# PhucNguyenAH/tacotron2_subword

Measured on AMD Instinct MI355X. Metric: mel_frames_per_sec_train, higher is better.
Workload: dtype bf16; 1 GPU; BERT_Tacotron2 default hparams (SMA), full training iteration fwd+loss+bwd+clip+Adam, B=64/GPU, 100 phones, 60 sub-word tokens, 400 frames, 80-mel; global_batch=64, frames_per_item=400, parallelism=dp1, torch_ops=loss reductions, cat/transpose copies, persistent_chains=True, recurrent_steps_bf16=True

## Files before the change

### include/t2amd.h

```cpp
#ifndef T2AMD_H
#define T2AMD_H
#include <stddef.h>
#include <stdint.h>

#ifdef __cplusplus
extern "C" {
#endif

#define T2_ATTN_SMA 0
#define T2_ATTN_LSA 1
#define T2_ATTN_DCA 4
#define T2_ATTN_GMM 3
#define T2_ATTN_FWD2 2

enum {
    T2_SITE_PRENET1 = 1, T2_SITE_PRENET2 = 2, T2_SITE_PRENET1_SUB = 3, T2_SITE_PRENET2_SUB = 4,
    T2_SITE_ATT_H = 5, T2_SITE_ATT_C = 6, T2_SITE_ATT_H_SUB = 7, T2_SITE_ATT_C_SUB = 8,
    T2_SITE_DEC_H = 9, T2_SITE_DEC_C = 10, T2_SITE_NOISE = 11, T2_SITE_NOISE_SUB = 12,
    T2_SITE_ENC0 = 16,
    T2_SITE_ENCSUB0 = 20,
    T2_SITE_POSTNET0 = 24
};

const char* t2_last_error(void);
#define T2_ABI_VERSION 4
int t2_version(void);
int t2_chain_status(uint32_t* out_host );
int t2_chain_status_clear(void);
int t2_debug_report_abort(uint32_t code, void* stream);
int t2_debug_occupy(int workgroups, int milliseconds, void* stream);
int t2_chain_claimed(void);
int t2_set_precision(int mode);
int t2_get_precision(void);
int t2_gemm_counts(uint64_t* out_host , int reset);
int t2_set_gemm_split_min_mflop(int mflop);
int t2_set_split_steps(int on);
int t2_get_split_steps(void);
int t2_step_counts(uint64_t* out_host , int reset);
int t2_set_overlap(int on);
int t2_set_chain(int on);
int t2_get_chain(void);
int t2_set_chain_bwd(int on);
int t2_set_gemm_staging(int on);
int t2_set_gemm_fold(int on);
int t2_set_bn_fuse(int on);
int t2_get_bn_fuse(void);
int t2_bn_fuse_counts(uint64_t* out_host , int reset);
int t2_side_join(void* stream);
int t2_defer_counts(uint64_t* out_host , int reset);

typedef struct t2_dims {
    int n_mel;
    int prenet_dim;
    int enc_dim;
    int att_rnn_dim;
    int dec_rnn_dim;
    int att_dim;
    int loc_filters;
    int loc_kernel;
    int attention_kind;
    float p_att_dropout, p_dec_dropout, p_prenet_dropout;
    int n_streams;
    float score_mask_value, score_mask_value_sub;
    int score_mask_given;
} t2_dims;

typedef struct t2_attention_weights {
    const float* wq;
    const float* wm;
    const float* v;
    const float* loc_conv;
    const float* loc_dense;
    const float* mlp_b1;
    const float* mlp_w2;
    const float* mlp_b2;
    const float* dca_T;
    const float* dca_bT;
    const float* dca_P;
} t2_attention_weights;
typedef struct t2_lstm_weights { const float *w_ih, *w_hh, *b_ih, *b_hh; } t2_lstm_weights;
typedef struct t2_decoder_weights {
    const float *prenet_w1, *prenet_w2;
    const float *prenet_sub_w1, *prenet_sub_w2;
    t2_lstm_weights att, att_sub;
    t2_attention_weights attn, attn_sub;
    t2_lstm_weights dec;
    const float *proj_w, *proj_b;
    const float *gate_w, *gate_b;
} t2_decoder_weights;

typedef struct t2_decoder_layout {
    size_t total_floats;
    size_t x, p1, p2, p1s, p2s;
    size_t pm, pms;
    size_t prea, preas;
    size_t ga, gas;
    size_t cna, cnas, ca, cas;
// ... 622 lines not shown
```

### tacotron2_subword_amd/_lib.py

```python
from __future__ import annotations

import ctypes as C
import os

import torch

_HERE = os.path.dirname(os.path.abspath(__file__))
LIB_PATH = os.environ.get("T2AMD_LIB") or os.path.join(_HERE, "libt2amd.so")

ATTN_SMA, ATTN_LSA, ATTN_FWD2, ATTN_GMM, ATTN_DCA = 0, 1, 2, 3, 4

SITE = dict(PRENET1=1, PRENET2=2, PRENET1_SUB=3, PRENET2_SUB=4, ATT_H=5, ATT_C=6, ATT_H_SUB=7, ATT_C_SUB=8,
            DEC_H=9, DEC_C=10, NOISE=11, NOISE_SUB=12, ENC0=16, ENCSUB0=20, POSTNET0=24)

_fp = C.POINTER(C.c_float)
_ip = C.POINTER(C.c_int32)


class Dims(C.Structure):
    _fields_ = [("n_mel", C.c_int), ("prenet_dim", C.c_int), ("enc_dim", C.c_int), ("att_rnn_dim", C.c_int),
                ("dec_rnn_dim", C.c_int), ("att_dim", C.c_int), ("loc_filters", C.c_int), ("loc_kernel", C.c_int),
                ("attention_kind", C.c_int), ("p_att_dropout", C.c_float), ("p_dec_dropout", C.c_float),
                ("p_prenet_dropout", C.c_float), ("n_streams", C.c_int),
                ("score_mask_value", C.c_float), ("score_mask_value_sub", C.c_float), ("score_mask_given", C.c_int)]
# ... 361 lines not shown
class WaveglowBackwardArgs(C.Structure):
    _fields_ = [("B", C.c_int), ("T", C.c_int), ("n_mel", C.c_int), ("n_samples", C.c_long), ("packed", C.c_void_p), ("packed_bwd", C.c_void_p),
                ("saved", C.c_void_p), ("mel", C.c_void_p), ("audio", C.c_void_p), ("dz", C.c_void_p), ("dlog_s_host", C.POINTER(C.c_void_p)),
                ("workspace", C.c_void_p), ("grad", C.c_void_p), ("kernel_ms_host", C.POINTER(C.c_double))]


class WaveglowWeightGradArgs(C.Structure):
    _fields_ = [("B", C.c_int), ("M", C.c_int), ("nc", C.c_int), ("n_cond", C.c_int), ("L", C.c_int), ("taps", C.c_int), ("d", C.c_int),
                ("a_rows", C.c_int), ("x_rows", C.c_int),
                ("a", C.c_void_p), ("x", C.c_void_p), ("spect", C.c_void_p), ("dw_x", C.c_void_p), ("dw_spect", C.c_void_p), ("db", C.c_void_p),
                ("workspace", C.c_void_p), ("db2", C.c_void_p)]


class WaveglowStartBackwardArgs(C.Structure):
    _fields_ = [("B", C.c_int), ("nc", C.c_int), ("c", C.c_int), ("n_half", C.c_int), ("L", C.c_int), ("dx", C.c_void_p), ("w_start", C.c_void_p),
                ("audio_in", C.c_void_p), ("d_in", C.c_void_p), ("dw_start", C.c_void_p), ("db_start", C.c_void_p), ("workspace", C.c_void_p)]


class WaveglowHeadBackwardArgs(C.Structure):
    _fields_ = [("B", C.c_int), ("n_group", C.c_int), ("n_samples", C.c_long), ("d_in", C.c_void_p), ("audio", C.c_void_p), ("part", C.c_void_p),
                ("dw", C.c_void_p)]


class WaveglowGateBackwardArgs(C.Structure):
    _fields_ = [("B", C.c_int), ("nc", C.c_int), ("L", C.c_int), ("last", C.c_int), ("dx", C.c_void_p), ("d_out", C.c_void_p), ("w_rs", C.c_void_p),
                ("t", C.c_void_p), ("g", C.c_void_p), ("packed_ws", C.c_void_p), ("du", C.c_void_p), ("acts", C.c_void_p)]


class WaveglowConvBackwardArgs(C.Structure):
    _fields_ = [("B", C.c_int), ("nc", C.c_int), ("n_cond", C.c_int), ("L", C.c_int), ("d", C.c_int), ("first_dx", C.c_int), ("first_spect", C.c_int),
                ("du", C.c_void_p), ("w_in", C.c_void_p), ("w_cond", C.c_void_p), ("packed_ws", C.c_void_p), ("dx", C.c_void_p), ("d_spect", C.c_void_p)]


class WaveglowTailBackwardArgs(C.Structure):
    _fields_ = [("B", C.c_int), ("nc", C.c_int), ("n_half", C.c_int), ("L", C.c_int), ("n_peel", C.c_int), ("n_group", C.c_int), ("z_offset", C.c_int),
                ("out", C.c_void_p), ("w_end", C.c_void_p), ("b_end", C.c_void_p), ("audio_in", C.c_void_p), ("w_next", C.c_void_p), ("d_next", C.c_void_p),
                ("dz", C.c_void_p), ("dlog_s", C.c_void_p), ("d_out", C.c_void_p), ("d_in", C.c_void_p), ("part", C.c_void_p), ("dw_end", C.c_void_p),
                ("db_end", C.c_void_p), ("dw_next", C.c_void_p)]


class WaveglowUpsampleBackwardArgs(C.Structure):
    _fields_ = [("B", C.c_int), ("n_mel", C.c_int), ("T", C.c_int), ("n_group", C.c_int), ("n_samples", C.c_long),
                ("mel", C.c_void_p), ("d_spect", C.c_void_p), ("dw", C.c_void_p), ("db", C.c_void_p)]


WAVEGLOW_KERNELS = ("upsample", "start", "gated_conv", "res_skip", "couple")
WAVEGLOW_FORWARD_KERNELS = ("upsample", "start", "gated_conv", "res_skip", "head", "tail", "sums")
WAVEGLOW_BACKWARD_KERNELS = ("tail_backward", "gate_backward", "conv_backward", "cond_backward", "weight_grad", "weight_grad_reduce", "start_backward",
                             "upsample_backward")
WAVEGLOW_GATED, WAVEGLOW_RES_SKIP, WAVEGLOW_UPSAMPLE = 0, 1, 2

ABI_VERSION = 4

EXPORTS = ["t2_last_error", "t2_version", "t2_chain_status", "t2_chain_status_clear", "t2_debug_report_abort", "t2_debug_occupy", "t2_chain_claimed", "t2_set_precision", "t2_get_precision", "t2_gemm_counts", "t2_set_gemm_split_min_mflop", "t2_set_split_steps", "t2_get_split_steps", "t2_step_counts", "t2_set_overlap", "t2_set_chain", "t2_get_chain", "t2_set_chain_bwd", "t2_set_gemm_staging", "t2_set_gemm_fold", "t2_set_bn_fuse", "t2_get_bn_fuse", "t2_bn_fuse_counts", "t2_side_join", "t2_defer_counts", "t2_decoder_layout_query", "t2_decoder_forward", "t2_decoder_infer",
           "t2_decoder_bwd_layout_query", "t2_decoder_backward", "t2_decoder_pass_plan", "t2_prof_enable", "t2_prof_collect", "t2_adam_chunks", "t2_adam_step", "t2_adam_norm",
           "t2_conv_bn_forward", "t2_conv_bn_backward", "t2_embedding_forward", "t2_embedding_backward",
           "t2_lstm_seq_forward", "t2_lstm_seq_backward", "t2_lstm_seq_chain_ws_floats", "t2_gemm_ex", "t2_prof_gemm", "t2_gemm_plan", "t2_chain_plan", "t2_conv_handoff_plan", "t2_colsum", "t2_mask_btc",
           "t2_finalize_bct", "t2_mask_bt", "t2_gemm", "t2_rng_keep_mask", "t2_rng_normal",
           "t2_softdtw_plan", "t2_softdtw_dist", "t2_softdtw_forward", "t2_softdtw_backward", "t2_softdtw_dist_backward",
           "t2_ssim_plan", "t2_ssim_forward", "t2_ssim_backward",
           "t2_hifigan_plan", "t2_hifigan_pack", "t2_hifigan_forward", "t2_vocoder_packed_floats", "t2_vocoder_conv1d", "t2_vocoder_conv_transpose1d",
           "t2_stft_plan", "t2_stft_pack", "t2_stft_analysis", "t2_stft_synthesis", "t2_melspec_plan", "t2_melspec_pack", "t2_melspec",
           "t2_waveglow_plan", "t2_waveglow_pack", "t2_waveglow_infer", "t2_waveglow_packed_floats", "t2_waveglow_gated_conv", "t2_waveglow_res_skip",
           "t2_waveglow_upsample", "t2_waveglow_couple", "t2_waveglow_forward_plan", "t2_waveglow_forward", "t2_waveglow_logdet",
           "t2_waveglow_logdet_matrices", "t2_waveglow_head", "t2_waveglow_tail",
           "t2_waveglow_backward_plan", "t2_waveglow_grad_offsets", "t2_waveglow_pack_backward", "t2_waveglow_train_forward", "t2_waveglow_backward",
           "t2_waveglow_weight_grad_ws_floats", "t2_waveglow_weight_grad", "t2_waveglow_gate_backward", "t2_waveglow_conv_backward_packed_floats",
           "t2_waveglow_conv_backward", "t2_waveglow_tail_backward", "t2_waveglow_upsample_backward", "t2_waveglow_start_backward", "t2_waveglow_head_backward"]

_lib = None


def lib() -> C.CDLL:
    global _lib
    if _lib is None:
        if not os.path.exists(LIB_PATH):
            raise RuntimeError(f"{LIB_PATH} is missing: the HIP extension must be built (see __graft_entry__.build); "
                               "there is no CPU fallback for the product path")
        L = C.CDLL(LIB_PATH)
        L.t2_last_error.restype = C.c_char_p
        if L.t2_version() != ABI_VERSION:
            raise RuntimeError(f"{LIB_PATH} speaks ABI version {L.t2_version()}, this binding {ABI_VERSION}: rebuild the library "
                               "(the argument structs differ in size between versions)")
        L.t2_chain_status.argtypes = [C.POINTER(C.c_uint32)]
        L.t2_debug_report_abort.argtypes = [C.c_uint32, C.c_void_p]
        L.t2_debug_occupy.argtypes = [C.c_int, C.c_int, C.c_void_p]
        L.t2_gemm.argtypes = [C.c_void_p, C.c_void_p, C.c_void_p, C.c_int, C.c_int, C.c_int, C.c_long, C.c_long, C.c_long,
                              C.c_long, C.c_long, C.c_void_p, C.c_int, C.c_float, C.c_float, C.c_void_p, C.c_size_t,
                              C.c_int, C.c_void_p]
        L.t2_rng_keep_mask.argtypes = [C.c_uint64, C.c_uint32, C.c_uint32, C.c_float, C.c_void_p, C.c_void_p]
        L.t2_rng_normal.argtypes = [C.c_uint64, C.c_uint32, C.c_uint32, C.c_void_p, C.c_void_p]
        L.t2_decoder_layout_query.argtypes = [C.POINTER(Dims), C.c_int, C.c_int, C.c_int, C.c_int, C.POINTER(DecoderLayout)]
        L.t2_decoder_forward.argtypes = [C.POINTER(Dims), C.POINTER(DecoderWeights), C.POINTER(DecoderFwdArgs), C.c_void_p]
        L.t2_decoder_infer.argtypes = [C.POINTER(Dims), C.POINTER(DecoderWeights), C.POINTER(DecoderInferArgs), C.c_void_p]
        L.t2_decoder_bwd_layout_query.argtypes = [C.POINTER(Dims), C.c_int, C.c_int, C.c_int, C.c_int, C.POINTER(DecoderBwdLayout)]
        L.t2_decoder_backward.argtypes = [C.POINTER(Dims), C.POINTER(DecoderWeights), C.POINTER(DecoderGrads),
                                          C.POINTER(DecoderBwdArgs), C.c_void_p]
        L.t2_decoder_pass_plan.argtypes = [C.POINTER(Dims), C.c_int, C.c_int, C.c_int, C.c_int, C.c_int, C.POINTER(PassEnv), C.c_int, C.c_int,
                                           C.POINTER(DecoderPassPlanInfo)]
        L.t2_conv_bn_forward.argtypes = [C.POINTER(ConvBnArgs), C.c_void_p]
        L.t2_conv_bn_backward.argtypes = [C.POINTER(ConvBnBwdArgs), C.c_void_p]
        L.t2_embedding_forward.argtypes = [C.c_void_p, C.c_void_p, C.c_void_p, C.c_int, C.c_int, C.c_void_p]
        L.t2_embedding_backward.argtypes = [C.c_void_p, C.c_void_p, C.c_void_p, C.c_int, C.c_int, C.c_int, C.c_void_p]
        L.t2_lstm_seq_forward.argtypes = [C.POINTER(LstmSeqArgs), C.c_void_p]
        L.t2_lstm_seq_backward.argtypes = [C.POINTER(LstmSeqBwdArgs), C.c_void_p]
        L.t2_lstm_seq_chain_ws_floats.argtypes, L.t2_lstm_seq_chain_ws_floats.restype = [C.c_int, C.c_int, C.c_int, C.c_int], C.c_size_t
        L.t2_gemm_ex.argtypes = [C.POINTER(GemmArgs), C.c_void_p]
# ... 300 lines not shown
    if not info.covered:
        return dict(covered=False, reason=info.reason, reason_text=info.reason_text.decode())
    out = {n: getattr(info, n) for n in ("instance", "grid", "lds_bytes", "UT", "RT", "CS", "MT", "lds_Tc", "lds_Tin", "lds_Jp", "lds_Jm",
                                         "q_bytes", "total_bytes", "ws_bytes")}
    out.update(covered=True, reason=0, instance_name=info.instance_name.decode(), Jp=list(info.Jp), Jm=list(info.Jm),
               parts={info.part_name[i].decode(): (info.part_off[i], info.part_bytes[i]) for i in range(CHAIN_PARTS) if info.part_bytes[i]},
               clear=(info.clear_off, info.clear_bytes), pass_clear_bytes=list(info.pass_clear_bytes))
    return out


def decoder_pass_plan(dims: Dims, kind: str, B: int, T: int, Tin: int, Tsub: int, *, defer_weight_grads: bool = False, poll_every: int = 0,
                      precision: str = "f32", split_steps: bool = False, chain: bool = True, chain_bwd: bool = True, overlap: bool = True,
                      cus: int = 256, claimed: bool = True, no_resident: bool = False, saved_tiles: bool = False) -> dict:
    env = PassEnv(PRECISION_MODES[precision], int(split_steps), int(chain), int(chain_bwd), int(overlap), cus, int(claimed), int(no_resident),
                  int(saved_tiles))
    info = DecoderPassPlanInfo()
    check(lib().t2_decoder_pass_plan(C.byref(dims), PASS_KINDS[kind], B, T, Tin, Tsub, C.byref(env), int(defer_weight_grads), poll_every, C.byref(info)))

    def chain_of(c):
        out = dict(asked=bool(c.asked), on=bool(c.on), reason=c.reason, reason_text=c.reason_text.decode())
        if c.on:
            out.update(instance=c.instance, instance_name=c.instance_name.decode(), grid=c.grid)
        return out

    def carve_of(c):
        return dict(w_ih16=(c.w_ih16_off, c.w_ih16_bytes), dg16=(c.dg16_off, c.dg16_bytes), rest=(c.rest_off, c.rest_bytes), total=c.total_bytes)

    out = dict(kind=kind, layout=info.layout, use16=bool(info.use16), split=bool(info.split), pre16=bool(info.pre16), scratch=carve_of(info.scratch),
               chain_a=chain_of(info.chain_a), chain_b=chain_of(info.chain_b), chained=bool(info.chained), overlap=bool(info.overlap),
               bounds=list(info.bounds[:info.nbounds]))
    if kind == "backward":
        out.update(bwd_layout=info.bwd_layout, defer=bool(info.defer), share=bool(info.share), chunk_cast=bool(info.chunk_cast),
                   ddin_ws=(info.ddin_ws_off, info.ddin_ws_bytes), dec_wgrads=("chain_b", "tail")[info.dec_wgrads],
                   dec_wgrads_staged=bool(info.dec_wgrads_staged), tail_on_side=bool(info.tail_on_side), tail_share=bool(info.tail_share),
                   tail_scratch=carve_of(info.tail_scratch), nsplit=info.nsplit, lsa_chain=bool(info.lsa_chain), dq_parts=info.dq_parts)
    else:
        out.update(clear=("status", "teacher", "decode")[info.clear], saves_tiles=bool(info.saves_tiles), poison_words=info.poison_words)
    if kind == "infer":
        out.update(poll=info.poll, shadow_floats=info.shadow_floats)
    return out


def conv_handoff_plan(args: GemmArgs, **opts) -> dict:
    o, info, taken = GemmPlanOpts(**opts), GemmPlanInfo(), C.c_int(0)
    check(lib().t2_conv_handoff_plan(C.byref(args), C.byref(o), C.byref(taken), C.byref(info)))
    return dict(taken=bool(taken.value), kernel=info.kernel, name=info.name.decode(), split=bool(info.split), splitk=info.splitk,
                kchunks=info.kchunks, a_src=info.a_src, b_src=info.b_src, stage_bytes_a=info.stage_bytes_a, stage_bytes_b=info.stage_bytes_b)


def set_gemm_fold(on: bool) -> None:
    check(lib().t2_set_gemm_fold(1 if on else 0))


def set_bn_fuse(on: bool) -> None:
    check(lib().t2_set_bn_fuse(1 if on else 0))


def get_bn_fuse() -> bool:
    return bool(lib().t2_get_bn_fuse())


def bn_fuse_counts(reset: bool = False):
    out = (C.c_uint64 * 3)()
    check(lib().t2_bn_fuse_counts(out, int(bool(reset))))
    return tuple(int(v) for v in out)


def defer_counts(reset: bool = False):
    out = (C.c_uint64 * 2)()
    check(lib().t2_defer_counts(out, int(bool(reset))))
    return tuple(int(v) for v in out)


def set_gemm_split_min_mflop(mflop: int = -1) -> None:
    check(lib().t2_set_gemm_split_min_mflop(int(mflop)))


def softdtw_plan(B: int, N: int, M: int, gamma: float = 1.0, need_grad: bool = False) -> SoftDtwPlanInfo:
    info = SoftDtwPlanInfo()
    check(lib().t2_softdtw_plan(B, N, M, gamma, int(bool(need_grad)), C.byref(info)))
    return info


def ssim_plan(N: int, H: int, W: int, ws: int = 11, need_grad: int = 0) -> SsimPlanInfo:
    info = SsimPlanInfo()
    check(lib().t2_ssim_plan(N, H, W, ws, int(need_grad), C.byref(info)))
    return info


def ssim_image(t: torch.Tensor | None) -> SsimImage:
    if t is None:
        return SsimImage(None, 0, 0, 0)
    if not t.is_cuda or t.dtype != torch.float32 or t.dim() != 4:
        raise RuntimeError("t2amd: an SSIM image must be a 4-D fp32 tensor on the GPU")
    B, Cn = t.shape[0], t.shape[1]
    sb, sc, sh, sw = t.stride()
    if B > 1 and Cn > 1 and sb != Cn * sc:
        raise RuntimeError("t2amd: SSIM image planes must be evenly spaced over batch and channel")
    return SsimImage(t.data_ptr(), sc if Cn > 1 else sb, sh, sw)


def ssim_forward(args: SsimFwdArgs) -> None:
    check(lib().t2_ssim_forward(C.byref(args), stream()))


def ssim_backward(args: SsimBwdArgs) -> None:
# ... 75 lines not shown
```

### tacotron2_subword_amd/csrc/c_api.hip

```cpp
#include <fcntl.h>
#include <stdarg.h>
#include <stdio.h>
#include <sys/file.h>
#include <unistd.h>
#include <stdlib.h>
#include <string.h>

#include "../../include/t2amd.h"
#include "kernels.h"
#include "chain_plan.h"
#include "driver.h"

static thread_local char g_err[512] = "";

void t2_set_error(const char* fmt, ...) {
    va_list ap;
    va_start(ap, fmt);
    vsnprintf(g_err, sizeof(g_err), fmt, ap);
    va_end(ap);
}

#include <algorithm>
#include <mutex>
#include <vector>
// ... 136 lines not shown
    T2_REQUIRE(w, "t2_chain_status: no status block");
    for (int i = 0; i < 4; ++i) out_host[i] = __atomic_load_n(w + i, __ATOMIC_RELAXED);
    return 0;
}
int t2_chain_status_clear(void) {
    unsigned* w = chain_sticky_words();
    T2_REQUIRE(w, "t2_chain_status_clear: no status block");
    for (int i = 0; i < 4; ++i) __atomic_store_n(w + i, 0u, __ATOMIC_RELAXED);
    return 0;
}
int t2_debug_report_abort(uint32_t code, void* stream) {
    unsigned* w = chain_sticky_words();
    T2_REQUIRE(w, "t2_debug_report_abort: no status block");
    hipLaunchKernelGGL(status_report_kernel, dim3(1), dim3(64), 0, (hipStream_t)stream, w, code);
    T2_LAUNCH_CHECK();
    return 0;
}
int t2_chain_claimed(void) { return chain_device_claim() ? 1 : 0; }
int t2_debug_occupy(int workgroups, int milliseconds, void* stream) {
    T2_REQUIRE(workgroups >= 1 && workgroups <= 256 && milliseconds >= 1 && milliseconds <= 5000, "t2_debug_occupy: 1..256 workgroups, 1..5000 ms");
    unsigned* w = chain_sticky_words();
    T2_REQUIRE(w, "t2_debug_occupy: no status block");
    const size_t smem = 96 * 1024;
    T2_TRY_RC(t2_allow_dynamic_lds(reinterpret_cast<const void*>(occupy_kernel), smem));
    hipLaunchKernelGGL(occupy_kernel, dim3(workgroups), dim3(256), smem, (hipStream_t)stream, (unsigned long long)milliseconds * 100000ull, w + 8);
    T2_LAUNCH_CHECK();
    return 0;
}
int t2_set_precision(int mode) {
    T2_REQUIRE(mode >= 0 && mode <= 2, "t2_set_precision: mode must be 0 (fp32), 1 (bf16 operands) or 2 (split-bf16 large GEMMs), not %d", mode);
    set_precision(mode);
    return 0;
}
int t2_get_precision(void) { return get_precision(); }
int t2_set_gemm_split_min_mflop(int mflop) { set_gemm_split_min_mflop(mflop); return 0; }
int t2_gemm_counts(uint64_t* out_host, int reset) {
    T2_REQUIRE(out_host, "null argument");
    gemm_counts(out_host, reset);
    return 0;
}
int t2_set_split_steps(int on) { g_split_steps = on != 0; return 0; }
int t2_get_split_steps(void) { return g_split_steps; }
int t2_step_counts(uint64_t* out_host, int reset) {
    T2_REQUIRE(out_host, "null argument");
    for (int i = 0; i < 6; ++i) { out_host[i] = g_step_counts[i]; if (reset) g_step_counts[i] = 0; }
    return 0;
}
int t2_set_overlap(int on) { g_overlap = on != 0; return 0; }
int t2_set_chain(int on) { g_chain = on != 0; return 0; }
int t2_get_chain(void) { return g_chain; }
int t2_set_chain_bwd(int on) { g_chain_bwd = on != 0; return 0; }
int t2_set_gemm_staging(int on) { set_gemm_staging(on); return 0; }
int t2_set_gemm_fold(int on) { set_gemm_fold(on); return 0; }
int t2_set_bn_fuse(int on) { set_bn_fuse(on); return 0; }
int t2_get_bn_fuse(void) { return get_bn_fuse(); }
int t2_bn_fuse_counts(uint64_t* out_host, int reset) {
    T2_REQUIRE(out_host, "null argument");
    bn_fuse_counts(out_host, reset);
    return 0;
}
int t2_defer_counts(uint64_t* out_host, int reset) {
    T2_REQUIRE(out_host, "null argument");
    for (int i = 0; i < 2; ++i) { out_host[i] = g_defer_counts[i]; if (reset) g_defer_counts[i] = 0; }
    return 0;
}
int t2_side_join(void* stream) {
    Side* side = nullptr;
    T2_TRY(side_get(&side));
    hipEvent_t e;
    T2_TRY(side_event(*side, 0, &e));
    T2_CHECK_HIP(hipEventRecord(e, side->s));
    T2_CHECK_HIP(hipStreamWaitEvent((hipStream_t)stream, e, 0));
    return 0;
}

int t2_conv_bn_forward(const t2_conv_bn_args* a, void* stream) {
    T2_REQUIRE(a, "null argument");
    const size_t nw = (size_t)a->Cout * a->Cin * a->K;
    T2_REQUIRE(a->ws_floats >= nw + 128 * (size_t)a->Cout, "t2_conv_bn_forward: workspace too small");
    ConvBnFwd f{};
    f.x = a->x; f.B = a->B; f.T = a->T; f.Cin = a->Cin; f.Cout = a->Cout; f.K = a->K;
    f.w = a->w; f.bias = a->bias; f.gamma = a->gamma; f.beta = a->beta; f.run_mean = a->run_mean; f.run_var = a->run_var;
    f.training = a->training; f.eps = a->eps; f.act = a->act; f.drop_p = a->drop_p; f.seed = a->seed; f.site = a->site;
    f.residual = a->residual; f.z = a->z; f.mean = a->mean; f.invstd = a->invstd; f.var = a->var; f.y = a->y;
    f.wperm = a->ws; f.scratch = a->ws + align4(nw);
    const size_t used = align4(nw) + 128 * (size_t)a->Cout;
    if (a->ws_floats > used) { f.gemm_ws = a->ws + used; f.gemm_ws_bytes = (a->ws_floats - used) * sizeof(float); }
    f.handoff = a->handoff; f.x16 = static_cast<const __bf16*>(a->x16); f.y16 = static_cast<__bf16*>(a->y16);
    return conv_bn_fwd(f, (hipStream_t)stream);
}

int t2_conv_bn_backward(const t2_conv_bn_bwd_args* a, void* stream) {
    T2_REQUIRE(a, "null argument");
    const size_t nw = align4((size_t)a->Cout * a->Cin * a->K), ndz = align4((size_t)a->B * a->T * a->Cout), nsc = 128 * (size_t)a->Cout;
    T2_REQUIRE(a->ws_floats >= nw + ndz + nsc, "t2_conv_bn_backward: workspace too small");
    ConvBnBwd f{};
    f.x = a->x; f.B = a->B; f.T = a->T; f.Cin = a->Cin; f.Cout = a->Cout; f.K = a->K;
    f.w = a->w; f.gamma = a->gamma; f.beta = a->beta; f.z = a->z; f.mean = a->mean; f.invstd = a->invstd;
    f.training = a->training; f.eps = a->eps; f.act = a->act; f.drop_p = a->drop_p; f.seed = a->seed; f.site = a->site;
    f.dy = a->dy; f.dw = a->dw; f.dbias = a->dbias; f.dgamma = a->dgamma; f.dbeta = a->dbeta;
    f.dx = a->dx; f.dx_accumulate = a->dx_accumulate;
    f.dz = a->ws; f.wperm = a->ws + ndz; f.scratch = a->ws + ndz + nw;
    f.gemm_ws = a->ws + ndz + nw + nsc; f.gemm_ws_bytes = (a->ws_floats - (ndz + nw + nsc)) * sizeof(float);
    f.handoff = a->handoff; f.x16 = static_cast<const __bf16*>(a->x16);
    return conv_bn_bwd(f, (hipStream_t)stream);
}
// ... 415 lines not shown
```

### tacotron2_subword_amd/csrc/gemm_dispatch.hip

```cpp
#include "gemm_common.h"
#include <cstdlib>
#include <algorithm>

namespace t2 {

using namespace gemm_detail;

static int g_precision = 0;
static int env_int(const char* name, int dflt) { const char* v = getenv(name); return v && *v ? atoi(v) : dflt; }
static int g_stage = env_int("T2_GEMM_STAGE", 1);
void set_gemm_staging(int on) { g_stage = on != 0; }
static int g_fold = env_int("T2_GEMM_FOLD", 1);
void set_gemm_fold(int on) { g_fold = on != 0; }
int get_gemm_fold() { return g_fold; }
constexpr int kStageMin = 256;
constexpr int kSplitMinMflopDefault = 2147;
static double g_split_min_flop = 1e6 * kSplitMinMflopDefault;
void set_gemm_split_min_mflop(int mflop) { g_split_min_flop = 1e6 * (mflop < 0 ? kSplitMinMflopDefault : mflop); }
void set_precision(int p) { g_precision = p; }
int get_precision() { return g_precision; }
static uint64_t g_counts[4] = {0, 0, 0, 0};
void gemm_counts(uint64_t* out, int reset) {
    for (int i = 0; i < 4; ++i) { out[i] = g_counts[i]; if (reset) g_counts[i] = 0; }
}

namespace {

__global__ void splitk_reduce_kernel(GemmDesc d) {
    const long total = (long)d.batch * d.M * d.N;
    const RngKey key = rng_key(d.seed, d.site);
    with_col_map(d, [&](auto cmap) {
    for (long i = blockIdx.x * (long)blockDim.x + threadIdx.x; i < total; i += (long)gridDim.x * blockDim.x) {
        float acc = 0.f;
        int s = 0;
        for (; s + 8 <= d.splitk; s += 8) {
            float v[8];
#pragma unroll
            for (int j = 0; j < 8; ++j) v[j] = d.ws[(long)(s + j) * total + i];
#pragma unroll
            for (int j = 0; j < 8; ++j) acc += v[j];
        }
        if (s + 4 <= d.splitk) {
            float v[4];
#pragma unroll
            for (int j = 0; j < 4; ++j) v[j] = d.ws[(long)(s + j) * total + i];
#pragma unroll
            for (int j = 0; j < 4; ++j) acc += v[j];
            s += 4;
        }
        for (; s < d.splitk; ++s) acc += d.ws[(long)s * total + i];
        const int bz = (int)(i / ((long)d.M * d.N));
        const long rem = i - (long)bz * d.M * d.N;
        const int m = (int)(rem / d.N), n = (int)(rem % d.N);
        epilogue_store<decltype(cmap)::value>(d, d.C + (long)bz * d.bsC, m, n, acc, key);
    }
    });
}

inline size_t round256(size_t n) { return (n + 255) & ~(size_t)255; }

int check_gemm(const GemmDesc& d) {
    T2_REQUIRE(d.M > 0 && d.N > 0 && d.K > 0 && d.batch > 0, "gemm: bad shape M=%d N=%d K=%d batch=%d", d.M, d.N, d.K, d.batch);
    if (d.conv_a || d.conv_b) {
        T2_REQUIRE(d.conv_T > 0 && d.conv_C > 0 && d.conv_C % 4 == 0 && !(d.conv_a && d.conv_b), "gemm: bad implicit-conv operand (T=%d C=%d)", d.conv_T, d.conv_C);
        T2_REQUIRE(d.batch == 1, "gemm: implicit-conv operands need batch == 1");
        if (d.conv_a) T2_REQUIRE(d.K % d.conv_C == 0 && aligned16(d.A), "gemm: conv A operand: K=%d C=%d", d.K, d.conv_C);
        if (d.conv_b) T2_REQUIRE(d.N % d.conv_C == 0 && aligned16(d.B), "gemm: conv B operand: N=%d C=%d", d.N, d.conv_C);
    }
    T2_REQUIRE(d.conv_a || d.sam == 1 || d.sak == 1, "gemm: A needs one unit stride (sam=%ld sak=%ld)", d.sam, d.sak);
    T2_REQUIRE(d.conv_b || d.sbn == 1 || d.sbk == 1, "gemm: B needs one unit stride (sbn=%ld sbk=%ld)", d.sbn, d.sbk);
    T2_REQUIRE(d.ccol_mod >= 0 && d.ccol_mul >= 0 && (!d.ccol_mod || (d.N % d.ccol_mod == 0 && (long)d.ccol_mul * d.ccol_mod >= d.N && (long)d.ccol_mul * d.ccol_mod <= d.ldc)),
               "gemm: bad column map (N=%d mod=%d mul=%d)", d.N, d.ccol_mod, d.ccol_mul);
    T2_REQUIRE(!d.r1_m == !d.r1_n && (!d.r1_m || d.batch == 1), "gemm: the rank-1 addend needs both vectors and batch == 1");
    T2_REQUIRE(d.drop_p == 0.f || (d.batch == 1 && (long)d.M * d.N < (1l << 32)), "gemm: dropout epilogue needs batch==1 and M*N < 2^32");
    return 0;
}

int choose_splitk(const GemmDesc& d, bool tile256, long tiles, int kch, size_t ws_bytes) {
    if (!(d.ws && d.beta == 0.f)) return 1;
    int sp = 1;
    if (tile256) {
        const int nkt = kch / 4;
        if (d.splitk > 0) sp = std::min(d.splitk, std::max(1, nkt / 2));
        else if (tiles < 512) {
            double best = 0.0;
            for (int c = 1; c <= 16; ++c) {
                if (c > 1 && nkt / c < 16) break;
                const long wgs = tiles * c, rounds = (wgs + 255) / 256;
                const double eff = (double)wgs / (256.0 * rounds);
                if (eff > best * 1.05) { best = eff; sp = c; }
            }
        }
    } else if (d.splitk > 0) sp = d.splitk;
    else if (tiles < 512 && kch >= 64) sp = std::min((int)((1024 + tiles - 1) / tiles), kch / 16);
    const size_t per = (size_t)d.batch * d.M * d.N * sizeof(float);
    if ((size_t)sp * per > ws_bytes) sp = (int)(ws_bytes / per);
    return std::max(sp, 1);
}

int run_gemm(const GemmDesc& d, const GemmPlan& p, hipStream_t s) {
    GemmK g{};
    g.d = d;
    g.kchunks = p.kchunks; g.avec = p.avec; g.bvec = p.bvec;
    if (d.conv_a) { g.d.sam = 0; g.d.sak = 1; }
    if (d.conv_b) { g.d.sbk = 0; g.d.sbn = 1; }
    if (d.drop_mstride == 0) g.d.drop_mstride = (uint32_t)d.N;
    g.d.K = p.K; g.d.conv_C = p.conv_C; g.d.splitk = p.splitk;
    const size_t staged = p.a.bytes + p.b.bytes;
    if (staged) { g.d.ws = reinterpret_cast<float*>(reinterpret_cast<unsigned char*>(d.ws) + staged); g.d.ws_bytes = d.ws_bytes - staged; }
    const int tile = p.kernel == GemmKernel::f32_64 ? 64 : p.kernel >= GemmKernel::src256 ? 256 : 128;
    const dim3 grid((d.N + tile - 1) / tile, (d.M + tile - 1) / tile, d.batch * p.splitk);
    if (gemm_reads_bf16_copies(p.kernel)) {
        __bf16* a16 = reinterpret_cast<__bf16*>(d.ws), * b16 = reinterpret_cast<__bf16*>(reinterpret_cast<unsigned char*>(d.ws) + p.a.bytes);
        if (p.a.src == GemmSrc::staged) T2_TRY_RC(stage_planned(d.A, p.a, p.split, a16, s));
        if (p.b.src == GemmSrc::staged) T2_TRY_RC(stage_planned(d.B, p.b, p.split, b16, s));
        const __bf16* pa = p.a.src == GemmSrc::caller ? d.A16 : a16, * pb = p.b.src == GemmSrc::caller ? d.B16 : b16;
        T2_TRY_RC(launch_gemm_bf16src(g, p.kernel, pa, p.a.ld, pb, p.b.ld, grid, s));
    } else if (p.kernel == GemmKernel::bf16conv) {
        T2_TRY_RC(launch_gemm_bf16conv(g, grid, s));
    } else {
        T2_TRY_RC(launch_gemm_f32(g, p.kernel, grid, s));
    }
    if (p.splitk > 1) {
        const long total = (long)d.batch * d.M * d.N;
        int blocks = (int)((total + 255) / 256);
        if (blocks > 2048) blocks = 2048;
        hipLaunchKernelGGL(splitk_reduce_kernel, dim3(blocks), dim3(256), 0, s, g.d);
        T2_LAUNCH_CHECK();
    }
    return 0;
}

}

const char* gemm_plan_name(const GemmPlan& p) {
    static const char* const names[] = {"f32_64", "f32_128", "bf16conv", "src128", "src256", "src256km", "x3src128", "x3src256", "x3src256km"};
    return names[(int)p.kernel + (p.split ? 3 : 0)];
}

GemmPlan plan_gemm(const GemmDesc& d) {
    GemmPlan p{};
    const bool conv_any = d.conv_a || d.conv_b;
    const bool akc = d.conv_a || d.sak == 1, bkc = !d.conv_b && d.sbk == 1;
    const long lda = d.conv_a ? d.conv_C : akc ? d.sam : d.sak;
    const long ldb = d.conv_b ? d.conv_C : bkc ? d.sbn : d.sbk;
    p.avec = aligned16(d.A) && d.bsA % 4 == 0 && lda % 4 == 0;
    p.bvec = aligned16(d.B) && d.bsB % 4 == 0 && ldb % 4 == 0;
    p.K = d.K; p.conv_C = d.conv_C;

    const bool large = !d.fp32_only && d.M >= 64 && d.N >= 64 && d.K >= 64 && (!conv_any || d.conv_C % 8 == 0);
    const bool use_bf16 = g_precision == 1 && large;
    const bool want_split = g_precision == 2 && large && 2.0 * d.M * d.N * d.K >= g_split_min_flop;
    const int kmul = want_split ? 3 : 1;
    const bool copies = g_precision != 2 || (want_split && d.split16);
    bool a_caller = copies && d.A16, b_caller = copies && d.B16;
    static const int g_t256 = env_int("T2_GEMM_256", 1);
    const bool shape256 = g_t256 && d.M % 256 == 0 && d.N % 256 == 0 && d.K >= 128;
    const long ld_km = std::max(std::max((long)d.M, a_caller && d.a16_kmajor ? d.lda16 : 0l), std::max((long)(d.conv_b ? d.conv_C : d.N), b_caller && d.b16_kmajor ? d.ldb16 : 0l));
    const bool km = shape256 && !akc && !bkc && !d.conv_a && (!d.conv_b || d.conv_C % 256 == 0) && (long)d.K * kmul * ld_km * 2 < (1l << 31);
    a_caller = a_caller && (d.a16_kmajor != 0) == km;
    b_caller = b_caller && (d.b16_kmajor != 0) == km;
    a_caller = a_caller && (!d.conv_a || d.lda16 == d.conv_C);
    const bool conv_ok = !conv_any || (d.conv_a && d.conv_C % 64 == 0 && (!want_split || (!a_caller && !b_caller))) ||
                         (d.conv_b && km && (!want_split || d.K % d.conv_T == 0));
    bool staged = false;
    size_t ws_bytes = d.ws_bytes;
    if ((use_bf16 || want_split) && g_stage && conv_ok && d.batch == 1 && d.M % 128 == 0 && d.N % 128 == 0 && d.K % 64 == 0) {
        const size_t a_elems = d.conv_a ? (size_t)d.M * d.conv_C : (size_t)d.M * d.K;
        const size_t b_elems = d.conv_b ? (size_t)d.K * d.conv_C : (size_t)d.N * d.K;
        const size_t need_a = a_caller ? 0 : round256(kmul * a_elems * sizeof(__bf16));
        const size_t need_b = b_caller ? 0 : round256(kmul * b_elems * sizeof(__bf16));
        const bool big = (a_caller || d.N >= kStageMin) && (b_caller || d.M >= kStageMin);
        const bool ok_src = (a_caller ? aligned16(d.A16) && d.lda16 % 8 == 0 : p.avec != 0) && (b_caller ? aligned16(d.B16) && d.ldb16 % 8 == 0 : p.bvec != 0);
        if (big && ok_src && (need_a + need_b == 0 || (d.ws && aligned16(d.ws) && d.ws_bytes >= need_a + need_b))) {
            staged = true;
            p.a.bytes = need_a; p.b.bytes = need_b;
            ws_bytes -= need_a + need_b;
        }
    }
    p.split = want_split && staged;
// ... 67 lines not shown
```

### tacotron2_subword_amd/csrc/gemm_f32.hip

```cpp
#include "gemm_common.h"

namespace t2 {
namespace gemm_detail {
namespace {

template <int R, bool KC>
__device__ __forceinline__ void load_tile(const float* __restrict__ base, long srow, long sk, int row0, int nrows,
                                          int k0, int kend, int vec, ConvAddr cv, f32x4 (&regs)[R * 4 / 256]) {
    constexpr int NQ = R * 4 / 256;
    if (!cv.T && vec && row0 + R <= nrows && k0 + BK <= kend) {
#pragma unroll
        for (int i = 0; i < NQ; ++i) {
            const int q = threadIdx.x + i * 256;
            const float* p = KC ? base + (long)(row0 + (q >> 2)) * srow + k0 + (q & 3) * 4
                                : base + (long)(k0 + q / (R / 4)) * sk + row0 + (q % (R / 4)) * 4;
            regs[i] = *reinterpret_cast<const f32x4*>(p);
        }
        return;
    }
#pragma unroll
    for (int i = 0; i < NQ; ++i) {
        int q = threadIdx.x + i * 256;
        f32x4 v = {0.f, 0.f, 0.f, 0.f};
        if (KC) {
// ... 71 lines not shown
    const int kbeg = split * g.kchunks * BK;
    const int kend = min(d.K, kbeg + g.kchunks * BK);

    const int lane = threadIdx.x & 63, wave = threadIdx.x >> 6;
    const int wm = wave >> 1, wn = wave & 1;
    const int r = lane & 31, hk = lane >> 5;

    f32x16 acc[TM][TN];
    zero(acc);

    const ConvAddr cva{d.conv_a ? d.conv_T : 0, d.conv_C, d.conv_pad}, cvb{d.conv_b ? d.conv_T : 0, d.conv_C, d.conv_pad};
    f32x4 ra[BM * 4 / 256], rb[BN * 4 / 256];
    if (kbeg < kend) {
        load_tile<BM, A_KC>(A, d.sam, d.sak, m0, d.M, kbeg, kend, g.avec, cva, ra);
        load_tile<BN, B_KC>(B, d.sbn, d.sbk, n0, d.N, kbeg, kend, g.bvec, cvb, rb);
        store_tile<BM, A_KC>(As[0], ra);
        store_tile<BN, B_KC>(Bs[0], rb);
    }
    __syncthreads();
    int cur = 0;
    for (int k0 = kbeg; k0 < kend; k0 += BK) {
        const bool more = k0 + BK < kend;
        if (more) {
            load_tile<BM, A_KC>(A, d.sam, d.sak, m0, d.M, k0 + BK, kend, g.avec, cva, ra);
            load_tile<BN, B_KC>(B, d.sbn, d.sbk, n0, d.N, k0 + BK, kend, g.bvec, cvb, rb);
        }
        const float* as = As[cur] + wm * (BM / 2) + r;
        const float* bs = Bs[cur] + wn * (BN / 2) + r;
#pragma unroll
        for (int kk = 0; kk < BK / 2; ++kk) {
            float a[TM], b[TN];
#pragma unroll
            for (int i = 0; i < TM; ++i) a[i] = as[(2 * kk + hk) * PA + i * 32];
#pragma unroll
            for (int j = 0; j < TN; ++j) b[j] = bs[(2 * kk + hk) * PB + j * 32];
#pragma unroll
            for (int i = 0; i < TM; ++i)
#pragma unroll
                for (int j = 0; j < TN; ++j)
                    acc[i][j] = __builtin_amdgcn_mfma_f32_32x32x2f32(a[i], b[j], acc[i][j], 0, 0, 0);
        }
        if (more) {
            store_tile<BM, A_KC>(As[cur ^ 1], ra);
            store_tile<BN, B_KC>(Bs[cur ^ 1], rb);
        }
        __syncthreads();
        cur ^= 1;
    }

    float* ws = d.splitk > 1 ? d.ws + ((long)split * d.batch + bz) * (long)d.M * d.N : nullptr;
    store_direct<true>(d, d.C + (long)bz * d.bsC, ws, acc, m0 + wm * (BM / 2), n0 + wn * (BN / 2), r, hk);
}

}

int launch_gemm_f32(const GemmK& g, GemmKernel kernel, dim3 grid, hipStream_t s) {
    using Kernel = void (*)(GemmK);
    static const Kernel f32_64[] = {gemm_kernel<64, 64, true, true>, gemm_kernel<64, 64, true, false>, gemm_kernel<64, 64, false, true>, gemm_kernel<64, 64, false, false>};
    static const Kernel f32_128[] = {gemm_kernel<128, 128, true, true>, gemm_kernel<128, 128, true, false>, gemm_kernel<128, 128, false, true>, gemm_kernel<128, 128, false, false>};
    const Kernel k = (kernel == GemmKernel::f32_64 ? f32_64 : f32_128)[(g.d.sak == 1 ? 0 : 2) + (g.d.sbk == 1 ? 0 : 1)];
    hipLaunchKernelGGL(k, grid, dim3(256), 0, s, g);
    T2_LAUNCH_CHECK();
    return 0;
}

}
}
```

### tacotron2_subword_amd/csrc/kernels.h

```cpp
#pragma once
#include "common.h"

namespace t2 {

enum Act : int { ACT_NONE = 0, ACT_RELU = 1, ACT_TANH = 2 };

struct GemmDesc {
    const float* A; const float* B; float* C;
    int M, N, K;
    long sam, sak;
    long sbn, sbk;
    long ldc;
    int batch; long bsA, bsB, bsC;
    float alpha, beta;
    const float* bias1; const float* bias2;
    int act;
    float drop_p; uint64_t seed; uint32_t site;
    uint32_t drop_base, drop_mstride;
    float* ws; size_t ws_bytes;
    int splitk;
    int conv_a, conv_b, conv_T, conv_C, conv_pad;
    int fp32_only;
    const __bf16* A16; long lda16;
    const __bf16* B16; long ldb16;
    int a16_kmajor, b16_kmajor;
    int split16;
    int crow_mod; long crow_mul;
    int ccol_mod, ccol_mul;
    const float* r1_m; const float* r1_n;
};
inline GemmDesc gemm_desc() {
    GemmDesc d{}; d.batch = 1; d.alpha = 1.f; d.beta = 0.f; d.act = ACT_NONE; d.drop_p = 0.f; return d;
}
int gemm(const GemmDesc& d, hipStream_t s);

enum class GemmKernel : int {
    f32_64, f32_128,
    bf16conv,
    src128,
    src256,
    src256km
};
inline bool gemm_reads_bf16_copies(GemmKernel k) { return k >= GemmKernel::src128; }
enum class GemmSrc : int { fp32, staged, caller };
struct GemmOperandPlan {
    GemmSrc src;
    long ld;
    bool kc; long ld_src; int rows, K, lo_slot, row_group;
    size_t bytes;
};
struct GemmPlan {
    GemmKernel kernel;
    bool split;
    int splitk, kchunks;
    int K, conv_C;
    GemmOperandPlan a, b;
    int avec, bvec;
};
GemmPlan plan_gemm(const GemmDesc& d);
int gemm_plan(const GemmDesc& d, GemmPlan* out);
bool gemm_handoff(const GemmDesc& plain, const GemmDesc& offered, GemmPlan* plan = nullptr);
const char* gemm_plan_name(const GemmPlan& p);
int stage_planned(const float* src, const GemmOperandPlan& o, bool split, __bf16* dst, hipStream_t s);
int stage_bf16(const float* src, bool kc, long ld, __bf16* dst, int rows, int K, hipStream_t s);
int stage_split_bf16(const float* src, bool kc, long ld, __bf16* dst, int rows, int K, int lo_slot, int row_group, hipStream_t s);
void set_precision(int p);
int get_precision();
void gemm_counts(uint64_t* out, int reset);
void set_gemm_split_min_mflop(int mflop);
void set_gemm_staging(int on);
void set_gemm_fold(int on);
int get_gemm_fold();

constexpr int kMaxSeg = 6;
struct LstmSeg { const float* x; long ldx; const float* w; long ldw; int k; };
struct LstmStream {
    LstmSeg seg[kMaxSeg]; int nseg;
    const float* pre; long ldpre;
    const float* bias1; const float* bias2;
    const float* c_prev; long ldc_prev;
    float* gates; long ldgates;
    float* c_new; long ldc_new;
    float* h_out; long ldh_out;
    float* h_out2; long ldh_out2;
    float* c_out; long ldc_out;
    uint32_t site_h, site_c; uint32_t idx_base, idx_bstride;
    const int* lengths; int t;
    const float* wq; int A; float* qpart;
    const __bf16* x16; long ldx16; const __bf16* w16; long ldw16; int k16;
    __bf16* h16_out; long ldh16;
    __bf16* h16_out2; long ldh16_2;
    const float* xs; long ldxs; const __bf16* w16lo;
};
constexpr int kMaxLstmStreams = 4;
struct LstmStepDesc { LstmStream st[kMaxLstmStreams]; int nstreams; int B, H; float drop_p; uint64_t seed; };
enum LstmFamily : int { LSTM_EXACT = 0, LSTM_BF16 = 1, LSTM_SPLIT = 2 };
int lstm_step_fwd(const LstmStepDesc& d, hipStream_t s, int* family = nullptr);

struct LstmBwdStream {
    const float* dh1; long lddh1;
    const float* dh2; long lddh2;
    const float* part; int nparts; long part_stride; long ldpart; int part_col;
    const float* dq; long lddq; const float* wq; int A;
    int dq_parts;
    const float* gates; long ldgates;
    const float* c_new; long ldc_new;
    const float* c_prev; long ldc_prev;
    float* dc_state;
    float* dg; long lddg;
    __bf16* dg16;
    uint32_t site_h, site_c, idx_base, idx_bstride;
};
struct LstmBwdPointDesc { LstmBwdStream st[kMaxLstmStreams]; int nstreams; int B, H; float drop_p; uint64_t seed; int first; };
int lstm_bwd_pointwise(const LstmBwdPointDesc& d, hipStream_t s);

struct LstmBwdSeg { const float* w; long ldw; int ncols; };
struct LstmBwdGemmStream {
    const float* dg; long lddg; LstmBwdSeg seg[3]; int nseg; float* part;
    const __bf16* dg16; const __bf16* wt16;
    const __bf16* wt16lo;
};
struct LstmBwdGemmDesc { LstmBwdGemmStream st[kMaxLstmStreams]; int nstreams; int B, H4, KS, NC; };
int lstm_bwd_gemm(const LstmBwdGemmDesc& d, hipStream_t s, int* family = nullptr);
int lstm_bwd_ksplit(int H4);
int cast_rows_bf16(const float* src, long ld_src, __bf16* dst, long ld_dst, int R, int C, hipStream_t s);
// ... 346 lines not shown
```

Baseline: 1.066 million mel-frames/s.

## Add specialized GEMV kernels and vectorized split-K reduce for degenerate GEMMs

Routes fp32 GEMMs with N==1 or M==1 away from the 64x64 MFMA tile kernel into dedicated GEMV kernels: a row kernel that stages A/B through shared memory, and a column kernel with vectorized B loads. It also adds a float4 split-K reduction kernel that is used when the output is 16-byte aligned. The aim is to avoid wasting most of an MFMA tile on single-row or single-column products and to cut reduce-kernel overhead. Both paths are gated by a new T2_GEMM_SPECIAL flag, on by default. The new kernels are plain FMA code, so summation order may differ slightly from the MFMA path.

Result: no change. 1.073 million mel-frames/s (median of 6 runs) (+0.6%).

```diff
diff --git a/include/t2amd.h b/include/t2amd.h
--- a/include/t2amd.h
+++ b/include/t2amd.h
@@ -43,6 +43,7 @@
 int t2_set_chain_bwd(int on);
 int t2_set_gemm_staging(int on);
 int t2_set_gemm_fold(int on);
+int t2_set_gemm_special(int on);
 int t2_set_bn_fuse(int on);
 int t2_get_bn_fuse(void);
 int t2_bn_fuse_counts(uint64_t* out_host , int reset);
diff --git a/tacotron2_subword_amd/_lib.py b/tacotron2_subword_amd/_lib.py
--- a/tacotron2_subword_amd/_lib.py
+++ b/tacotron2_subword_amd/_lib.py
@@ -437,7 +437,7 @@
 
 ABI_VERSION = 4
 
-EXPORTS = ["t2_last_error", "t2_version", "t2_chain_status", "t2_chain_status_clear", "t2_debug_report_abort", "t2_debug_occupy", "t2_chain_claimed", "t2_set_precision", "t2_get_precision", "t2_gemm_counts", "t2_set_gemm_split_min_mflop", "t2_set_split_steps", "t2_get_split_steps", "t2_step_counts", "t2_set_overlap", "t2_set_chain", "t2_get_chain", "t2_set_chain_bwd", "t2_set_gemm_staging", "t2_set_gemm_fold", "t2_set_bn_fuse", "t2_get_bn_fuse", "t2_bn_fuse_counts", "t2_side_join", "t2_defer_counts", "t2_decoder_layout_query", "t2_decoder_forward", "t2_decoder_infer",
+EXPORTS = ["t2_last_error", "t2_version", "t2_chain_status", "t2_chain_status_clear", "t2_debug_report_abort", "t2_debug_occupy", "t2_chain_claimed", "t2_set_precision", "t2_get_precision", "t2_gemm_counts", "t2_set_gemm_split_min_mflop", "t2_set_split_steps", "t2_get_split_steps", "t2_step_counts", "t2_set_overlap", "t2_set_chain", "t2_get_chain", "t2_set_chain_bwd", "t2_set_gemm_staging", "t2_set_gemm_fold", "t2_set_gemm_special", "t2_set_bn_fuse", "t2_get_bn_fuse", "t2_bn_fuse_counts", "t2_side_join", "t2_defer_counts", "t2_decoder_layout_query", "t2_decoder_forward", "t2_decoder_infer",
            "t2_decoder_bwd_layout_query", "t2_decoder_backward", "t2_decoder_pass_plan", "t2_prof_enable", "t2_prof_collect", "t2_adam_chunks", "t2_adam_step", "t2_adam_norm",
            "t2_conv_bn_forward", "t2_conv_bn_backward", "t2_embedding_forward", "t2_embedding_backward",
            "t2_lstm_seq_forward", "t2_lstm_seq_backward", "t2_lstm_seq_chain_ws_floats", "t2_gemm_ex", "t2_prof_gemm", "t2_gemm_plan", "t2_chain_plan", "t2_conv_handoff_plan", "t2_colsum", "t2_mask_btc",
@@ -844,6 +844,10 @@
     check(lib().t2_set_gemm_fold(1 if on else 0))
 
 
+def set_gemm_special(on: bool) -> None:
+    check(lib().t2_set_gemm_special(1 if on else 0))
+
+
 def set_bn_fuse(on: bool) -> None:
     check(lib().t2_set_bn_fuse(1 if on else 0))
 
diff --git a/tacotron2_subword_amd/csrc/c_api.hip b/tacotron2_subword_amd/csrc/c_api.hip
--- a/tacotron2_subword_amd/csrc/c_api.hip
+++ b/tacotron2_subword_amd/csrc/c_api.hip
@@ -212,6 +212,7 @@
 int t2_set_chain_bwd(int on) { g_chain_bwd = on != 0; return 0; }
 int t2_set_gemm_staging(int on) { set_gemm_staging(on); return 0; }
 int t2_set_gemm_fold(int on) { set_gemm_fold(on); return 0; }
+int t2_set_gemm_special(int on) { set_gemm_special(on); return 0; }
 int t2_set_bn_fuse(int on) { set_bn_fuse(on); return 0; }
 int t2_get_bn_fuse(void) { return get_bn_fuse(); }
 int t2_bn_fuse_counts(uint64_t* out_host, int reset) {
diff --git a/tacotron2_subword_amd/csrc/gemm_dispatch.hip b/tacotron2_subword_amd/csrc/gemm_dispatch.hip
--- a/tacotron2_subword_amd/csrc/gemm_dispatch.hip
+++ b/tacotron2_subword_amd/csrc/gemm_dispatch.hip
@@ -13,6 +13,9 @@
 static int g_fold = env_int("T2_GEMM_FOLD", 1);
 void set_gemm_fold(int on) { g_fold = on != 0; }
 int get_gemm_fold() { return g_fold; }
+static int g_special = env_int("T2_GEMM_SPECIAL", 1);
+void set_gemm_special(int on) { g_special = on != 0; }
+int get_gemm_special() { return g_special; }
 constexpr int kStageMin = 256;
 constexpr int kSplitMinMflopDefault = 2147;
 static double g_split_min_flop = 1e6 * kSplitMinMflopDefault;
@@ -55,6 +58,47 @@
         epilogue_store<decltype(cmap)::value>(d, d.C + (long)bz * d.bsC, m, n, acc, key);
     }
     });
+}
+
+__global__ __launch_bounds__(256) void splitk_reduce4_kernel(GemmDesc d) {
+    const long total = (long)d.batch * d.M * d.N;
+    const long i = (blockIdx.x * 256l + threadIdx.x) * 4;
+    if (i >= total) return;
+    const f32x4* p = reinterpret_cast<const f32x4*>(d.ws + i);
+    const long plane = total / 4;
+    f32x4 acc = {0.f, 0.f, 0.f, 0.f};
+    int s = 0;
+    for (; s + 16 <= d.splitk; s += 16) {
+        f32x4 v[16];
+#pragma unroll
+        for (int j = 0; j < 16; ++j) v[j] = p[(long)(s + j) * plane];
+#pragma unroll
+        for (int j = 0; j < 16; ++j) acc += v[j];
+    }
+    if (s < d.splitk) {
+        const int left = d.splitk - s;
+        f32x4 v[16];
+#pragma unroll
+        for (int j = 0; j < 16; ++j) if (j < left) v[j] = p[(long)(s + j) * plane];
+#pragma unroll
+        for (int j = 0; j < 16; ++j) if (j < left) acc += v[j];
+    }
+    int bz, m, n;
+    if (total < (1l << 31)) {
+        const unsigned row = (unsigned)i / (unsigned)d.N;
+        n = (int)((unsigned)i - row * (unsigned)d.N);
+        bz = d.batch > 1 ? (int)(row / (unsigned)d.M) : 0;
+        m = (int)(row - (unsigned)bz * (unsigned)d.M);
+    } else {
+        const long row = i / d.N;
+        n = (int)(i - row * d.N);
+        bz = (int)(row / d.M);
+        m = (int)(row - (long)bz * d.M);
+    }
+    const RngKey key = rng_key(d.seed, d.site);
+    float* C = d.C + (long)bz * d.bsC;
+#pragma unroll
+    for (int c = 0; c < 4; ++c) epilogue_store<false>(d, C, m, n + c, acc[c], key);
 }
 
 inline size_t round256(size_t n) { return (n + 255) & ~(size_t)255; }
@@ -123,9 +167,14 @@
     }
     if (p.splitk > 1) {
         const long total = (long)d.batch * d.M * d.N;
-        int blocks = (int)((total + 255) / 256);
-        if (blocks > 2048) blocks = 2048;
-        hipLaunchKernelGGL(splitk_reduce_kernel, dim3(blocks), dim3(256), 0, s, g.d);
+        const long blocks4 = (total / 4 + 255) / 256;
+        if (g_special && d.N % 4 == 0 && d.ldc % 4 == 0 && !d.ccol_mod && aligned16(d.C) && aligned16(g.d.ws) && blocks4 < (1l << 31)) {
+            hipLaunchKernelGGL(splitk_reduce4_kernel, dim3((unsigned)blocks4), dim3(256), 0, s, g.d);
+        } else {
+            int blocks = (int)((total + 255) / 256);
+            if (blocks > 2048) blocks = 2048;
+            hipLaunchKernelGGL(splitk_reduce_kernel, dim3(blocks), dim3(256), 0, s, g.d);
+        }
         T2_LAUNCH_CHECK();
     }
     return 0;
diff --git a/tacotron2_subword_amd/csrc/gemm_f32.hip b/tacotron2_subword_amd/csrc/gemm_f32.hip
--- a/tacotron2_subword_amd/csrc/gemm_f32.hip
+++ b/tacotron2_subword_amd/csrc/gemm_f32.hip
@@ -147,9 +147,166 @@
     store_direct<true>(d, d.C + (long)bz * d.bsC, ws, acc, m0 + wm * (BM / 2), n0 + wn * (BN / 2), r, hk);
 }
 
+__device__ __forceinline__ float pad_chunk(float acc, int klen) { return klen % BK ? acc + 0.0f : acc; }
+
+constexpr int GV_R = 64, GV_KT = 128, GV_P = GV_KT + 4, GV_NQ = GV_R * GV_KT / 4 / 256;
+
+__global__ __launch_bounds__(256) void gemv_rows_kernel(GemmK g) {
+    const GemmDesc& d = g.d;
+    __shared__ __attribute__((aligned(16))) float As[2][GV_R * GV_P];
+    __shared__ __attribute__((aligned(16))) float Bs[2][GV_KT];
+
+    const int z = blockIdx.z;
+    const int split = z % d.splitk, bz = z / d.splitk;
+    const float* A = d.A + (long)bz * d.bsA;
+    const float* B = d.B + (long)bz * d.bsB;
+    const int m0 = blockIdx.x * GV_R;
+    const int kbeg = split * g.kchunks * BK;
+    const int kend = min(d.K, kbeg + g.kchunks * BK);
+    const int tid = threadIdx.x;
+
+    f32x4 ra[GV_NQ];
+    float rb = 0.f;
+    auto load = [&](int k0) {
+#pragma unroll
+        for (int i = 0; i < GV_NQ; ++i) {
+            const int q = tid + i * 256;
+            const int row = m0 + (q >> 5), k = k0 + (q & 31) * 4;
+            f32x4 v = {0.f, 0.f, 0.f, 0.f};
+            if (row < d.M && k < kend) {
+                const float* p = A + (long)row * d.sam + k;
+                if (g.avec && k + 3 < kend) {
+                    v = *reinterpret_cast<const f32x4*>(p);
+                } else {
+#pragma unroll
+                    for (int j = 0; j < 4; ++j) if (k + j < kend) v[j] = p[j];
+                }
+            }
+            ra[i] = v;
+        }
+        if (tid < GV_KT) rb = k0 + tid < kend ? B[(long)(k0 + tid) * d.sbk] : 0.f;
+    };
+    auto store = [&](int buf) {
+#pragma unroll
+        for (int i = 0; i < GV_NQ; ++i) {
+            const int q = tid + i * 256;
+            *reinterpret_cast<f32x4*>(&As[buf][(q >> 5) * GV_P + (q & 31) * 4]) = ra[i];
+        }
+        if (tid < GV_KT) Bs[buf][tid] = rb;
+    };
+
+    if (kbeg < kend) { load(kbeg); store(0); }
+    __syncthreads();
+    float acc = 0.f;
+    int cur = 0;
+    for (int k0 = kbeg; k0 < kend; k0 += GV_KT) {
+        const bool more = k0 + GV_KT < kend;
+        if (more) load(k0 + GV_KT);
+        if (tid < GV_R) {
+            const int nch = (min(kend - k0, GV_KT) + BK - 1) / BK;
+            const float* as = &As[cur][tid * GV_P];
+            const float* bs = Bs[cur];
+            for (int c = 0; c < nch; ++c) {
+#pragma unroll
+                for (int q = 0; q < BK / 4; ++q) {
+                    const f32x4 a = *reinterpret_cast<const f32x4*>(as + c * BK + q * 4);
+                    const f32x4 b = *reinterpret_cast<const f32x4*>(bs + c * BK + q * 4);
+#pragma unroll
+                    for (int j = 0; j < 4; ++j) acc = fmaf(a[j], b[j], acc);
+                }
+            }
+        }
+        if (more) store(cur ^ 1);
+        __syncthreads();
+        cur ^= 1;
+    }
+
+    const int m = m0 + tid;
+    if (tid >= GV_R || m >= d.M) return;
+    if (d.splitk > 1) {
+        d.ws[((long)split * d.batch + bz) * (long)d.M * d.N + (long)m * d.N] = acc;
+    } else {
+        const RngKey key = rng_key(d.seed, d.site);
+        with_col_map(d, [&](auto cmap) { epilogue_store<decltype(cmap)::value>(d, d.C + (long)bz * d.bsC, m, 0, acc, key); });
+    }
+}
+
+template <int V, int U>
+__global__ __launch_bounds__(64) void gemv_cols_kernel(GemmK g) {
+    const GemmDesc& d = g.d;
+    typedef float vec __attribute__((ext_vector_type(V)));
+    const int z = blockIdx.z;
+    const int split = z % d.splitk, bz = z / d.splitk;
+    const int n = (blockIdx.x * 64 + threadIdx.x) * V;
+    if (n >= d.N) return;
+    const float* A = d.A + (long)bz * d.bsA;
+    const float* B = d.B + (long)bz * d.bsB + n;
+    const int kbeg = split * g.kchunks * BK;
+    const int kend = min(d.K, kbeg + g.kchunks * BK);
+
+    float acc[V];
+#pragma unroll
+    for (int c = 0; c < V; ++c) acc[c] = 0.f;
+    int k = kbeg;
+    for (; k + U <= kend; k += U) {
+        vec v[U];
+        float a[U];
+#pragma unroll
+        for (int j = 0; j < U; ++j) v[j] = *reinterpret_cast<const vec*>(B + (long)(k + j) * d.sbk);
+#pragma unroll
+        for (int j = 0; j < U; ++j) a[j] = A[(long)(k + j) * d.sak];
+#pragma unroll
+        for (int j = 0; j < U; ++j)
+#pragma unroll
+            for (int c = 0; c < V; ++c) acc[c] = fmaf(a[j], v[j][c], acc[c]);
+    }
+    if (k < kend) {
+        const int left = kend - k;
+        vec v[U];
+        float a[U];
+#pragma unroll
+        for (int j = 0; j < U; ++j)
+            if (j < left) { v[j] = *reinterpret_cast<const vec*>(B + (long)(k + j) * d.sbk); a[j] = A[(long)(k + j) * d.sak]; }
+#pragma unroll
+        for (int j = 0; j < U; ++j)
+            if (j < left)
+#pragma unroll
+                for (int c = 0; c < V; ++c) acc[c] = fmaf(a[j], v[j][c], acc[c]);
+    }
+#pragma unroll
+    for (int c = 0; c < V; ++c) acc[c] = pad_chunk(acc[c], max(kend - kbeg, 0));
+
+    if (d.splitk > 1) {
+        float* ws = d.ws + ((long)split * d.batch + bz) * (long)d.M * d.N + n;
+#pragma unroll
+        for (int c = 0; c < V; ++c) ws[c] = acc[c];
+    } else {
+        const RngKey key = rng_key(d.seed, d.site);
+        with_col_map(d, [&](auto cmap) {
+#pragma unroll
+            for (int c = 0; c < V; ++c) epilogue_store<decltype(cmap)::value>(d, d.C + (long)bz * d.bsC, 0, n + c, acc[c], key);
+        });
+    }
+}
+
 }
 
 int launch_gemm_f32(const GemmK& g, GemmKernel kernel, dim3 grid, hipStream_t s) {
+    const GemmDesc& d = g.d;
+    if (kernel == GemmKernel::f32_64 && get_gemm_special() && !d.conv_a && !d.conv_b) {
+        if (d.N == 1 && d.sak == 1) {
+            hipLaunchKernelGGL(gemv_rows_kernel, dim3((d.M + GV_R - 1) / GV_R, 1, grid.z), dim3(256), 0, s, g);
+            T2_LAUNCH_CHECK();
+            return 0;
+        }
+        if (d.M == 1 && d.sbn == 1) {
+            const long waves4 = (long)((d.N + 255) / 256) * grid.z;
+            if (g.bvec && d.N % 4 == 0 && waves4 >= 1024) hipLaunchKernelGGL((gemv_cols_kernel<4, 16>), dim3((d.N + 255) / 256, 1, grid.z), dim3(64), 0, s, g);
+            else hipLaunchKernelGGL((gemv_cols_kernel<1, 32>), dim3((d.N + 63) / 64, 1, grid.z), dim3(64), 0, s, g);
+            T2_LAUNCH_CHECK();
+            return 0;
+        }
+    }
     using Kernel = void (*)(GemmK);
     static const Kernel f32_64[] = {gemm_kernel<64, 64, true, true>, gemm_kernel<64, 64, true, false>, gemm_kernel<64, 64, false, true>, gemm_kernel<64, 64, false, false>};
     static const Kernel f32_128[] = {gemm_kernel<128, 128, true, true>, gemm_kernel<128, 128, true, false>, gemm_kernel<128, 128, false, true>, gemm_kernel<128, 128, false, false>};
diff --git a/tacotron2_subword_amd/csrc/kernels.h b/tacotron2_subword_amd/csrc/kernels.h
--- a/tacotron2_subword_amd/csrc/kernels.h
+++ b/tacotron2_subword_amd/csrc/kernels.h
@@ -71,6 +71,8 @@
 void set_gemm_staging(int on);
 void set_gemm_fold(int on);
 int get_gemm_fold();
+void set_gemm_special(int on);
+int get_gemm_special();
 
 constexpr int kMaxSeg = 6;
 struct LstmSeg { const float* x; long ldx; const float* w; long ldw; int k; };
```
